# codelion/adaptive-classifier

Hardware: AMD Instinct MI355X
Metric: predict() queries/sec + kNN GB/s vs HBM roofline, 768-d (higher is better)
Workload: dtype f32

## Files before the change

### adaptive-classifier_amd/csrc/bert.hip

```cpp
#include "common.h"
#include "attention_core.h"

#include <math.h>
#include <atomic>
#include <chrono>
#include <string.h>

namespace {

typedef float f32x4 __attribute__((ext_vector_type(4)));
constexpr int kMaxVec = 8;

__device__ __forceinline__ float wave_sum(float v) {
#pragma unroll
    for (int o = 1; o < 64; o <<= 1) v += __shfl_xor(v, o);
    return v;
}

template <bool F16 = false>
__device__ __forceinline__ void layernorm_store(f32x4 (&x)[kMaxVec], int H, int lane, const float* g,
                                                const float* b, float eps, float* dst, uint16_t* planes = nullptr,
                                                int64_t rows = 0, int64_t row = 0) {
    const int nv = H >> 2;
    float s = 0.f;
// ... 4 lines not shown
    float q = 0.f;
#pragma unroll
    for (int e = 0; e < kMaxVec; ++e)
        if (lane + 64 * e < nv) {
            const float d0 = x[e].x - mean, d1 = x[e].y - mean, d2 = x[e].z - mean, d3 = x[e].w - mean;
            q += (d0 * d0 + d1 * d1) + (d2 * d2 + d3 * d3);
        }
    const float var = wave_sum(q) / (float)H;
    const float rstd = 1.0f / sqrtf(var + eps);
#pragma unroll
    for (int e = 0; e < kMaxVec; ++e) {
        const int c4 = lane + 64 * e;
        if (c4 < nv) {
            const f32x4 gg = *reinterpret_cast<const f32x4*>(g + 4 * c4);
            const f32x4 bb = *reinterpret_cast<const f32x4*>(b + 4 * c4);
            f32x4 y;
            y.x = (x[e].x - mean) * rstd * gg.x + bb.x;
            y.y = (x[e].y - mean) * rstd * gg.y + bb.y;
            y.z = (x[e].z - mean) * rstd * gg.z + bb.z;
            y.w = (x[e].w - mean) * rstd * gg.w + bb.w;
            *reinterpret_cast<f32x4*>(dst + 4 * c4) = y;
            if (planes)
                ac::emit_planes4(planes + ac::plane_off(rows, row, 4 * c4), rows * (int64_t)H, y, F16);
        }
    }
}

template <bool F16>
__global__ __launch_bounds__(256) void embed_ln_kernel(const int64_t* ids, const int64_t* type_ids, int T, int S,
                                                       int H, const float* word, const float* pos,
                                                       const float* type, const float* g, const float* b,
                                                       float eps, float* out, uint16_t* planes,
                                                       const int32_t* __restrict__ tok_src = nullptr,
                                                       const int32_t* __restrict__ t_dev = nullptr) {
    if (t_dev) T = t_dev[0];
    const int lane = threadIdx.x & 63;
    const int t = blockIdx.x * 4 + (threadIdx.x >> 6);
    if (t >= T) return;
    const int src = tok_src ? tok_src[t] : t;
    const int64_t id = ids[src];
    const int64_t tt = type_ids ? type_ids[src] : 0;
    const int p = src % S;
    const int nv = H >> 2;
    f32x4 x[kMaxVec];
#pragma unroll
    for (int e = 0; e < kMaxVec; ++e) {
        const int c4 = lane + 64 * e;
        if (c4 < nv) {
            const f32x4 w = *reinterpret_cast<const f32x4*>(word + id * H + 4 * c4);
            if (type) {
                const f32x4 ty = *reinterpret_cast<const f32x4*>(type + tt * H + 4 * c4);
                const f32x4 po = *reinterpret_cast<const f32x4*>(pos + (int64_t)p * H + 4 * c4);
                x[e] = (w + ty) + po;
            } else {
                x[e] = w;
            }
        }
    }
    layernorm_store<F16>(x, H, lane, g, b, eps, out + (int64_t)t * H, planes, T, t);
}

template <bool F16>
__global__ __launch_bounds__(256) void ln_kernel_t(const float* in, int T, int H, const float* g, const float* b,
                                                   float eps, float* out, uint16_t* planes, int64_t in_stride) {
    const int lane = threadIdx.x & 63;
    const int t = blockIdx.x * 4 + (threadIdx.x >> 6);
    if (t >= T) return;
// ... 582 lines not shown
    return AC_OK;
}

}

extern "C" int ac_bert_workspace(const ac_bert_config* cfg, int b, int S, size_t* bytes) {
    int rc = check_cfg(cfg);
    if (rc) return rc;
    AC_REQUIRE(bytes && b >= 0 && S >= 1, AC_EINVAL, "bert workspace: bad arguments");
    *bytes = bert_ws(*cfg, b > 0 ? b : 1, S).total;
    return AC_OK;
}

namespace {

static bool tail_fused() {
    const char* e = getenv("AC_BERT_TAIL_FUSED");
    return !(e && atoi(e) == 0);
}
inline bool pools_mean(int pool_opt) { return pool_opt == AC_POOL_MEAN; }
inline int token_layers(const ac_bert_config& c) { return pools_mean(c.pool_opt) ? c.layers : c.layers - 1; }
struct EncodePlan { bool wplanes, pl, f16; };
EncodePlan encode_plan(const ac_bert_config& c, const ac_bert_weights* w, int T) {
    const int H = c.hidden, I = c.intermediate;
    EncodePlan p;
    p.wplanes = w->qkv_w3 && w->ao_w3 && w->ff1_w3 && w->ff2_w3;
    p.pl = p.wplanes && ac::linear_takes_planes(T, H, H) && ac::linear_takes_planes(T, H, I) && (H % 8) == 0;
    p.f16 = p.pl && ac::gemm_arith() == AC_GEMM_F16X2 && w->qkv_wh && w->ao_wh && w->ff1_wh && w->ff2_wh && token_layers(c) > 0 &&
            ac::linear_f16x2_takes(T, 3 * H, H) && ac::linear_f16x2_takes(T, H, H) && ac::linear_f16x2_takes(T, I, H) &&
            ac::linear_f16x2_takes(T, H, I);
    return p;
}
void launch_embed(const ac_bert_config& c, const ac_bert_weights* w, const EncodePlan& pn, const int64_t* d_ids, const int64_t* d_type_ids,
                  int rows, int S, float* x, uint16_t* xp, const int32_t* tok_src, const int32_t* t_dev, hipStream_t stream) {
    const int H = c.hidden, tok_blocks = (rows + 3) / 4;
    if (pn.f16)
        hipLaunchKernelGGL(embed_ln_kernel<true>, dim3(tok_blocks), dim3(256), 0, stream, d_ids, d_type_ids, rows, S, H,
                           w->word_emb, w->pos_emb, w->type_emb, w->emb_ln_g, w->emb_ln_b, c.ln_eps, x, xp, tok_src, t_dev);
    else
        hipLaunchKernelGGL(embed_ln_kernel<false>, dim3(tok_blocks), dim3(256), 0, stream, d_ids, d_type_ids, rows, S, H,
                           w->word_emb, w->pos_emb, w->type_emb, w->emb_ln_g, w->emb_ln_b, c.ln_eps, x,
                           pn.pl ? xp : nullptr, tok_src, t_dev);
}
constexpr int kPreCtl = 1, kPreEmbed = 2;
int bert_encode_impl(const ac_bert_config* cfg, const ac_bert_weights* w, const int64_t* d_ids, const int64_t* d_type_ids,
                     const int64_t* d_mask, int b, int S, const int32_t* cu, const int32_t* tok_src, int T, int Smax,
                     float* d_out, int64_t ldo, void* d_ws, size_t ws_bytes, hipStream_t stream, int pre = 0) {
    int rc;
    const ac_bert_config& c = *cfg;
    const BertWs ws = bert_ws(c, b, S);
    AC_REQUIRE(d_ws && ws_bytes >= ws.total, AC_EWORKSPACE, "bert_encode_cls: workspace %zu < %zu", ws_bytes, ws.total);
    char* base = (char*)d_ws;
    float* x = (float*)(base + ws.x);
    float* qkv = (float*)(base + ws.qkv);
    float* ctx = (float*)(base + ws.ctx);
    float* y = (float*)(base + ws.y);
    float* ffn = (float*)(base + ws.ffn);
    const int H = c.hidden, I = c.intermediate;

    uint16_t* xp = (uint16_t*)(base + ws.xp);
    uint16_t* ctxp = (uint16_t*)(base + ws.ctxp);
    uint16_t* ffnp = (uint16_t*)(base + ws.ffnp);
    const EncodePlan pn = encode_plan(c, w, T);
    const bool wplanes = pn.wplanes, pl = pn.pl;
    const bool f16 = pn.f16;
    const bool pool = pools_mean(c.pool_opt);
    const bool fuse_ln = pl && token_layers(c) > 0 && ac::pipe_ln_applies(T, H, H) && ac::pipe_ln_applies(T, H, I);
    unsigned* ln_abort = (unsigned*)base;
    if (!(pre & kPreCtl)) {
        hipLaunchKernelGGL(ln_verdict_roll_kernel, dim3(1), dim3(1), 0, stream, ln_abort);
        AC_LAUNCH_CHECK();
    }
    unsigned* ln_count = (unsigned*)(base + ws.lnctl);
    const int ln_panels = ac::pipe_ln_panels(T);
    if (fuse_ln && !(pre & kPreCtl)) AC_HIP_CHECK(hipMemsetAsync(base + ws.lnctl, 0, ws.lnctl_bytes, stream));

    if (!(pre & kPreEmbed)) {
        launch_embed(c, w, pn, d_ids, d_type_ids, T, S, x, xp, tok_src, nullptr, stream);
        AC_LAUNCH_CHECK();
    }
    const int dh = c.hidden / c.heads;
    const float scale = 1.0f / sqrtf((float)dh);
    const int32_t* cu_at = cu;
    const bool fuse_attn = pl && token_layers(c) > 0 && dh == 64 && (cu || !d_mask) && ac::qkv_attn_applies(T, H, c.heads, Smax);
    if (fuse_attn && !cu) {
        int32_t* cuw = (int32_t*)(base + ws.cu);
        hipLaunchKernelGGL(iota_cu_kernel, dim3((b + 256) / 256), dim3(256), 0, stream, cuw, b, S);
        AC_LAUNCH_CHECK();
        cu_at = cuw;
    }
    int32_t* tile_seq = (int32_t*)(base + ws.tile_seq);
    unsigned* attn_xchg = nullptr;
    if (fuse_attn) {
        if (!(pre & kPreCtl) || !cu) {
            rc = ac::qkv_attn_tile_seq(cu_at, b, T, tile_seq, stream);
            if (rc) return rc;
        }
        if (ac::qkv_attn_exchange_applies(T, c.heads, (int)f16)) {
            attn_xchg = (unsigned*)(base + ws.attn_xchg);
            if (!(pre & kPreCtl)) AC_HIP_CHECK(hipMemsetAsync(attn_xchg, 0, ws.attn_xchg_bytes, stream));
        }
    }
    for (int l = 0; l < c.layers; ++l) {
        const uint16_t* qkv_w3 = wplanes ? w->qkv_w3[l] : nullptr;
        const uint16_t* ao_w3 = wplanes ? w->ao_w3[l] : nullptr;
        const uint16_t* ff1_w3 = wplanes ? w->ff1_w3[l] : nullptr;
        const uint16_t* ff2_w3 = wplanes ? w->ff2_w3[l] : nullptr;
        const bool last = (l == c.layers - 1) && !pool;
        const int Ml = last ? b : T;
        const bool lp = pl && !last;
        const float* resid = x;
// ... 25 lines not shown
            rc = ac::linear_f32_splitk(resid, ldres, w->qkv_w[l], H, w->qkv_b[l], nullptr, 0, y, H, b, H, H, 0, qkv_w3, ctx,
                                       (size_t)T * H * sizeof(float), stream, 3 * H);
        } else {
            rc = f16 ? ac::linear_f16x2(xp, w->qkv_wh[l], w->qkv_b[l], nullptr, 0, qkv, 3 * H, nullptr, T, 3 * H, H, 0, stream)
                     : ac::linear_f32(x, H, w->qkv_w[l], H, w->qkv_b[l], nullptr, 0, qkv, 3 * H, T, 3 * H, H, 0, nullptr, 1.f,
                                      stream, 0.f, 0, qkv_w3, pl ? xp : nullptr);
        }
        if (rc) return rc;
        if (fuse_attn && !last) {
        } else if (last) {
            const float* qc = q_cls_only ? y : nullptr;
            if (dh == 64 && Smax <= 32)
                hipLaunchKernelGGL((attention_cls_kernel<false, 64, 32>), dim3(c.heads, b), dim3(64), 0, stream, qkv, d_mask, S, H, scale,
                                   ctx, nullptr, nullptr, -1, cu, qc);
            else if (dh == 64)
                hipLaunchKernelGGL((attention_cls_kernel<false, 64>), dim3(c.heads, b), dim3(64), 0, stream, qkv, d_mask, S, H, scale,
                                   ctx, nullptr, nullptr, -1, cu, qc);
            else
                hipLaunchKernelGGL((attention_cls_kernel<false, 32>), dim3(c.heads, b), dim3(64), 0, stream, qkv, d_mask, S, H, scale,
                                   ctx, nullptr, nullptr, -1, cu, qc);
        } else {
            if (dh == 64)
                hipLaunchKernelGGL((attention_mfma_kernel<false, 64>), dim3((Smax + 31) / 32, c.heads, b), dim3(64), 0, stream, qkv,
                                   d_mask, S, H, scale, ctx, lp ? ctxp : nullptr, nullptr, nullptr, -1, cu, (int64_t)T, (int)f16);
            else
                hipLaunchKernelGGL((attention_mfma_kernel<false, 32>), dim3((Smax + 31) / 32, c.heads, b), dim3(64), 0, stream, qkv,
                                   d_mask, S, H, scale, ctx, lp ? ctxp : nullptr, nullptr, nullptr, -1, cu, (int64_t)T, (int)f16);
        }
        AC_LAUNCH_CHECK();
        const int lblocks = (Ml + 3) / 4;
        const bool fl = fuse_ln && lp;
        if (fl) {
            rc = ac::launch_gemm_pipe_ln(ctxp, Ml, f16 ? w->ao_wh[l] : ao_w3, H, w->ao_b[l], x, H, x, H, Ml, H, H, w->ln1_g[l], w->ln1_b[l], c.ln_eps,
                                         base + ws.lnpart, ln_count + (size_t)(2 * l) * ln_panels, ln_abort, xp, stream, (int)f16);
            if (rc) return rc;
        } else {
            rc = last ? ac::linear_f32_splitk(ctx, H, w->ao_w[l], H, w->ao_b[l], resid, ldres, y, H, Ml, H, H, 0, ao_w3, qkv,
                                              (size_t)T * 3 * H * sizeof(float), stream)
                      : (f16 ? ac::linear_f16x2(ctxp, w->ao_wh[l], w->ao_b[l], resid, ldres, y, H, nullptr, Ml, H, H, 0, stream)
                             : ac::linear_f32(ctx, H, w->ao_w[l], H, w->ao_b[l], resid, ldres, y, H, Ml, H, H, 0, nullptr, 1.f, stream,
                                              0.f, 0, ao_w3, lp ? ctxp : nullptr));
            if (rc) return rc;
            launch_ln(f16, lblocks, stream, y, Ml, H, w->ln1_g[l], w->ln1_b[l], c.ln_eps, last ? ctx : x, lp ? xp : nullptr, (int64_t)H);
            AC_LAUNCH_CHECK();
        }
        float* x1 = last ? ctx : x;
        rc = last ? ac::linear_f32_splitk(x1, H, w->ff1_w[l], H, w->ff1_b[l], nullptr, 0, ffn, I, Ml, I, H, 2, ff1_w3, qkv,
                                          (size_t)T * 3 * H * sizeof(float), stream)
                  : (f16 ? ac::linear_f16x2(xp, w->ff1_wh[l], w->ff1_b[l], nullptr, 0, nullptr, I, ffnp, Ml, I, H, 2, stream)
                         : ac::linear_f32(x1, H, w->ff1_w[l], H, w->ff1_b[l], nullptr, 0, ffn, I, Ml, I, H, 2, nullptr, 1.f, stream,
                                          0.f, 0, ff1_w3, lp ? xp : nullptr, lp ? ffnp : nullptr));
        if (rc) return rc;
        if (fl) {
            rc = ac::launch_gemm_pipe_ln(ffnp, Ml, f16 ? w->ff2_wh[l] : ff2_w3, H, w->ff2_b[l], x, H, x, H, Ml, H, I, w->ln2_g[l], w->ln2_b[l], c.ln_eps,
                                         base + ws.lnpart, ln_count + (size_t)(2 * l + 1) * ln_panels, ln_abort, xp, stream, (int)f16);
            if (rc) return rc;
            continue;
        }
        if (last && tail_fused()) {
            int ks = 0;
            rc = ac::linear_f32_splitk(ffn, I, w->ff2_w[l], I, w->ff2_b[l], x1, H, y, H, Ml, H, I, 0, ff2_w3, qkv,
                                       (size_t)T * 3 * H * sizeof(float), stream, 0, &ks);
            if (rc) return rc;
            if (ks > 0) {
                hipLaunchKernelGGL(splitk_ln_normalize_kernel, dim3(b), dim3(64), 0, stream, qkv, ks, b, H, w->ff2_b[l], x1, (int64_t)H,
                                   w->ln2_g[l], w->ln2_b[l], c.ln_eps, d_out, ldo);
                AC_LAUNCH_CHECK();
                return AC_OK;
            }
            launch_ln(f16, lblocks, stream, y, Ml, H, w->ln2_g[l], w->ln2_b[l], c.ln_eps, x, nullptr, (int64_t)H);
            AC_LAUNCH_CHECK();
            break;
        }
        rc = last ? ac::linear_f32_splitk(ffn, I, w->ff2_w[l], I, w->ff2_b[l], x1, H, y, H, Ml, H, I, 0, ff2_w3, qkv,
                                          (size_t)T * 3 * H * sizeof(float), stream)
                  : (f16 ? ac::linear_f16x2(ffnp, w->ff2_wh[l], w->ff2_b[l], x1, H, y, H, nullptr, Ml, H, I, 0, stream)
                         : ac::linear_f32(ffn, I, w->ff2_w[l], I, w->ff2_b[l], x1, H, y, H, Ml, H, I, 0, nullptr, 1.f, stream, 0.f, 0,
                                          ff2_w3, lp ? ffnp : nullptr));
        if (rc) return rc;
        launch_ln(f16, lblocks, stream, y, Ml, H, w->ln2_g[l], w->ln2_b[l], c.ln_eps, x, lp ? xp : nullptr, (int64_t)H);
        AC_LAUNCH_CHECK();
    }
    if (pool) {
        hipLaunchKernelGGL(pool_mean_normalize_kernel<false>, dim3(b), dim3(256), 3 * (size_t)H * sizeof(float), stream, x, d_mask, cu, S, H,
                           (const float*)nullptr, (const float*)nullptr, 0.f, d_out, ldo);
        AC_LAUNCH_CHECK();
        return AC_OK;
    }
// ... 89 lines not shown
    *epoch_out = (int)(n & 0x3fffffff) + 1;
    return base ? base + 16 * (n & 63) : nullptr;
}
}

static std::atomic<long long> g_unpad_wait_ns{0};
extern "C" long long ac_bert_unpad_last_wait_ns(void) { return g_unpad_wait_ns.load(std::memory_order_relaxed); }

extern "C" int ac_bert_encode_cls_unpad(const ac_bert_config* cfg, const ac_bert_weights* w, const int64_t* d_ids,
                                        const int64_t* d_type_ids, const int64_t* d_mask, int b, int S, float* d_out, int64_t ldo,
                                        void* d_ws, size_t ws_bytes, int clear_verdict, int* total_tokens, int* path, ac_stream_t stream_) {
    if (total_tokens) *total_tokens = 0;
    if (path) *path = AC_BERT_PATH_PACKED;
    int rc = check_cfg(cfg);
    if (rc) return rc;
    if (b == 0) return AC_OK;
    hipStream_t stream = (hipStream_t)stream_;
    const ac::CallScope scope(cfg->gemm_arith_opt, cfg->ln_fusion_opt, cfg->one_launch_opt);
    AC_REQUIRE(w && d_ids && d_mask && d_out && b > 0 && S >= 2 && S <= cfg->max_pos && ldo >= cfg->hidden && (int64_t)b * S > 32 &&
                   (int64_t)b * S < ((int64_t)1 << 30),
               AC_EINVAL, "bert_encode_cls_unpad: bad arguments (b=%d S=%d max_pos=%d; more than 32 token rows)", b, S, cfg->max_pos);
    const ac_bert_config& c = *cfg;
    const BertWs ws = bert_ws(c, b, S);
    AC_REQUIRE(d_ws && ws_bytes >= ws.total, AC_EWORKSPACE, "bert_encode_cls_unpad: workspace %zu < %zu", ws_bytes, ws.total);
    char* base = (char*)d_ws;
    int32_t* cu = (int32_t*)(base + ws.cu);
    int32_t* src = (int32_t*)(base + ws.pack_src);
    int32_t* info = (int32_t*)(base + ws.pack_info);
    int epoch = 0;
    int32_t* slot = info_slot(&epoch);
    const size_t lds = (size_t)(2 * b + 1) * sizeof(int32_t);
    AC_REQUIRE(slot && lds <= 96 * 1024, AC_EUNSUPPORTED, "bert_encode_cls_unpad: %d sequences in one call (or no pinned host memory): "
               "use ac_bert_pack + ac_bert_encode_cls_packed", b);
    if (lds > 48 * 1024) (void)hipFuncSetAttribute((const void*)pack_prologue_kernel, hipFuncAttributeMaxDynamicSharedMemorySize, (int)lds);
    hipLaunchKernelGGL(pack_prologue_kernel, dim3(1), dim3(1024), lds, stream, d_mask, b, S, cu, src, info, (int32_t*)(base + ws.tile_seq),
                       (unsigned*)(base + ws.lnctl), (int)(ws.lnctl_bytes / 4), (unsigned*)(base + ws.attn_xchg), (int)(ws.attn_xchg_bytes / 4),
                       (unsigned*)base, clear_verdict, slot, epoch);
    AC_LAUNCH_CHECK();
    const EncodePlan lo = encode_plan(c, w, b), hi = encode_plan(c, w, b * S);
    const bool early = lo.pl == hi.pl && lo.f16 == hi.f16;
    if (early) {
        launch_embed(c, w, hi, d_ids, d_type_ids, b * S, S, (float*)(base + ws.x), (uint16_t*)(base + ws.xp), src, info, stream);
        AC_LAUNCH_CHECK();
    }
    volatile int32_t* vs = slot;
    bool seen = false;
    const auto wait_t0 = std::chrono::steady_clock::now();
    for (int spin = 0; spin < 200000 && !seen; ++spin) {
        seen = __atomic_load_n(&vs[3], __ATOMIC_ACQUIRE) == epoch;
        if (!seen) __builtin_ia32_pause();
    }
    if (!seen) {
        AC_HIP_CHECK(hipStreamSynchronize(stream));
        seen = __atomic_load_n(&vs[3], __ATOMIC_ACQUIRE) == epoch;
        AC_REQUIRE(seen, AC_EHIP, "bert_encode_cls_unpad: the packing kernel's report never arrived");
    }
    g_unpad_wait_ns.store(std::chrono::duration_cast<std::chrono::nanoseconds>(std::chrono::steady_clock::now() - wait_t0).count(),
                          std::memory_order_relaxed);
    const int total = vs[0], not_prefix = vs[1], longest = vs[2];
    if (total_tokens) *total_tokens = total;
    if (!not_prefix && total < b * S) {
        AC_REQUIRE(total >= b && longest >= 1 && longest <= S, AC_EHIP, "bert_encode_cls_unpad: bad report (%d rows, longest %d)", total, longest);
        return bert_encode_impl(cfg, w, d_ids, d_type_ids, nullptr, b, S, cu, src, total, longest, d_out, ldo, d_ws, ws_bytes, stream,
                                kPreCtl | (early ? kPreEmbed : 0));
    }
    if (path) *path = not_prefix ? AC_BERT_PATH_PADDED_MASK : AC_BERT_PATH_PADDED;
    if (total_tokens) *total_tokens = b * S;
    return bert_encode_impl(cfg, w, d_ids, d_type_ids, not_prefix ? d_mask : nullptr, b, S, nullptr, nullptr, b * S, S, d_out, ldo, d_ws,
                            ws_bytes, stream);
}

extern "C" int ac_bert_encode_cls_packed(const ac_bert_config* cfg, const ac_bert_weights* w, const int64_t* d_ids,
                                         const int64_t* d_type_ids, int b, int S, const int32_t* d_cu,
                                         const int32_t* d_tok_src, int total_tokens, int longest, float* d_out, int64_t ldo,
                                         void* d_ws, size_t ws_bytes, ac_stream_t stream_) {
// ... 194 lines not shown
```

### adaptive-classifier_amd/csrc/common.h

```cpp
#pragma once
#include <atomic>
#include <hip/hip_runtime.h>
#include <stdarg.h>
#include <stdint.h>
#include <stdio.h>

#include "../../include/acamd.h"

namespace ac {

void set_error(const char* fmt, ...);

struct DevInfo {
    int cus;
    int lds_per_block;
    size_t hbm_bytes;
    int hw_cus;
};
const DevInfo& dev_info();

bool test_hooks_enabled();
#define AC_TEST_HOOK_ONLY(name)                                                                                                   \
    do {                                                                                                                          \
        if (!ac::test_hooks_enabled()) {                                                                                          \
// ... 16 lines not shown

#define AC_REQUIRE(cond, code, ...)                                                     \
    do {                                                                                \
        if (!(cond)) {                                                                  \
            ac::set_error(__VA_ARGS__);                                                 \
            return (code);                                                              \
        }                                                                               \
    } while (0)

#define AC_LAUNCH_CHECK()                                                               \
    do {                                                                                \
        hipError_t _e = hipGetLastError();                                              \
        if (_e != hipSuccess) {                                                         \
            ac::set_error("kernel launch failed: %s (%s:%d)", hipGetErrorString(_e),    \
                          __FILE__, __LINE__);                                          \
            return AC_EHIP;                                                             \
        }                                                                               \
    } while (0)

__host__ __device__ static inline size_t align_up(size_t x, size_t a) { return (x + a - 1) / a * a; }
static inline int next_pow2(int x) { int p = 1; while (p < x) p <<= 1; return p; }

int linear_f32(const float* A, int64_t lda, const float* W, int64_t ldw, const float* bias,
               const float* residual, int64_t ldr, float* C, int64_t ldc, int M, int N, int K, int act,
               const uint8_t* mask, float mask_scale, hipStream_t stream, float drop_p = 0.f,
               uint64_t drop_seed = 0, const uint16_t* W_planes = nullptr, const uint16_t* A_planes = nullptr,
               uint16_t* C_planes = nullptr, int64_t w_plane_rows = 0);
int linear_f32_splitk(const float* A, int64_t lda, const float* W, int64_t ldw, const float* bias, const float* residual,
                      int64_t ldr, float* C, int64_t ldc, int M, int N, int K, int act, const uint16_t* W_planes, float* scratch,
                      size_t scratch_bytes, hipStream_t stream, int64_t w_plane_rows = 0, int* partials_only = nullptr);
bool pipe_ln_applies(int M, int N, int K);
size_t pipe_ln_part_bytes(int M, int N);
int pipe_ln_panels(int M);
int launch_gemm_pipe_ln(const uint16_t* Ap, int64_t a_rows, const uint16_t* Wp, int64_t w_rows, const float* bias,
                        const float* residual, int64_t ldr, float* C, int64_t ldc, int M, int N, int K, const float* gamma,
                        const float* beta, float eps, void* part, unsigned* count, unsigned* abort_flag, uint16_t* planes,
                        hipStream_t stream, int f16 = 0);
constexpr int kQkvAttnRows = 256;
constexpr int kQkvAttnCu = 264;
bool qkv_attn_applies(int M, int H, int heads, int smax);
size_t qkv_attn_tile_seq_bytes(int M);
int qkv_attn_tile_seq(const int32_t* cu, int b, int M, int32_t* tile_seq, hipStream_t stream);
bool qkv_attn_exchange_applies(int M, int heads, int f16);
int launch_gemm_pipe_qkv_attn(const uint16_t* Ap, int64_t a_rows, const uint16_t* Wp, int64_t w_rows, const float* bias, int M, int H,
                              int heads, const int32_t* cu, const int32_t* tile_seq, int b, int smax, float scale, uint16_t* ctx_planes,
                              float* qkv, hipStream_t stream, int f16 = 0, unsigned* exchange = nullptr, unsigned epoch = 0,
                              unsigned* abort_flag = nullptr);
bool linear_takes_planes(int M, int N, int K);

__host__ __device__ static inline bool dropout_keep(uint64_t seed, uint64_t idx, float p) {
    uint64_t z = seed + idx * 0x9E3779B97F4A7C15ull;
    z = (z ^ (z >> 30)) * 0xBF58476D1CE4E5B9ull;
    z = (z ^ (z >> 27)) * 0x94D049BB133111EBull;
    z ^= z >> 31;
    return (float)(z >> 40) * (1.0f / 16777216.0f) >= p;
}
#ifdef __HIPCC__
typedef __bf16 bf16x2_t __attribute__((ext_vector_type(2)));
typedef float f32x2_t __attribute__((ext_vector_type(2)));
typedef float f32x4_t __attribute__((ext_vector_type(4)));

__device__ __forceinline__ uint32_t pack_bf16(float a, float b) {
    const f32x2_t f = {a, b};
    return __builtin_bit_cast(uint32_t, __builtin_convertvector(f, bf16x2_t));
}
__device__ __forceinline__ void split2(float a, float b, uint32_t& h, uint32_t& m, uint32_t& l) {
    h = pack_bf16(a, b);
    const float ra = a - __uint_as_float(h << 16), rb = b - __uint_as_float(h & 0xffff0000u);
    m = pack_bf16(ra, rb);
    const float sa = ra - __uint_as_float(m << 16), sb = rb - __uint_as_float(m & 0xffff0000u);
// ... 244 lines not shown
```

### adaptive-classifier_amd/csrc/gemm_common.h

```cpp
#pragma once
#include "common.h"
#include "gemm_plan.h"

#include <math.h>

namespace acg {

typedef float f32x4 __attribute__((ext_vector_type(4)));
typedef float f32x16 __attribute__((ext_vector_type(16)));

struct Epilogue {
    const float* bias = nullptr;
    const float* residual = nullptr;
    int64_t ldr = 0;
    int act = ACT_NONE;
    float alpha = 1.f;
    float beta = 0.f;
    const uint8_t* mask = nullptr;
    float mask_scale = 1.f;
    uint64_t drop_seed = 0;
    float drop_p = 0.f;
    const float* gate = nullptr;
    int64_t ldg = 0;
    float gate_scale = 1.f;
};

struct LnFuse {
    const float* gamma;
    const float* beta;
    float eps;
    float2* part;
    unsigned* count;
    unsigned* abort_;
    uint16_t* planes;
    int starve;
    int fences;
};

struct AttnFuse {
    const int32_t* cu;
    const int32_t* tile_seq;
    int b, H, smax;
    float scale;
    uint16_t* ctx_planes;
    float* qkv;
    unsigned* exchange;
    unsigned epoch;
    int fences;
    unsigned* abort_;
};

__device__ __forceinline__ float apply_epilogue(const Epilogue& e, float acc, int64_t row, int col,
                                                const float* C, int64_t ldc, int N) {
    float v = e.alpha * acc;
    if (e.beta != 0.f) v = fmaf(e.beta, C[row * ldc + col], v);
    if (e.bias) v += e.bias[col];
    if (e.act == ACT_RELU) v = v < 0.f ? 0.f : v;
    else if (e.act == ACT_GELU) v = ac::gelu_erf(v);
    if (e.mask) v = e.mask[row * (int64_t)N + col] ? v * e.mask_scale : 0.f;
    else if (e.drop_p > 0.f) v = ac::dropout_keep(e.drop_seed, (uint64_t)(row * (int64_t)N + col), e.drop_p) ? v * e.mask_scale : 0.f;
    if (e.residual) v += e.residual[row * e.ldr + col];
    if (e.gate) v = (e.gate[row * e.ldg + col] != 0.f) ? v * e.gate_scale : 0.f;
    return v;
}

template <int EPI>
__device__ __forceinline__ float fast_epilogue(float acc, float bias, float res) {
    if (EPI == EPI_IDENT) return acc;
// ... 132 lines not shown
```

### adaptive-classifier_amd/csrc/gemm_pipe.hip

```cpp
#include "common.h"
#include "gemm_common.h"
#include "grid_sync.h"
#include "attention_core.h"

#include <stdio.h>
#include <stdlib.h>

#include <atomic>
#include <type_traits>

namespace {
using namespace acg;

constexpr int PSBK = 16;

struct PipeParams {
    const uint16_t* Ap; int64_t a_rows;
    const uint16_t* Wp; int64_t w_rows;
    float* C; int64_t ldc;
    int M, N, K;
    Epilogue epi;
    LnFuse ln;
    AttnFuse at;
    unsigned long long* stamps;
    int krot;
};

template <int STRIDE = 4>
__device__ __forceinline__ void stamp(const PipeParams& prm, int wave, int i) {
    if (prm.stamps && wave == 0) {
        const unsigned long long t = clock64();
        if ((threadIdx.x & 63) == 0) prm.stamps[(size_t)blockIdx.x * STRIDE + i] = t;
    }
}

template <int N> __device__ __forceinline__ void wait_vm() {
    static_assert(N >= 0 && N <= 63, "vmcnt immediate");
    asm volatile("s_waitcnt vmcnt(%0)" ::"n"(N) : "memory");
}
// ... 37 lines not shown
    static_assert(BM <= 64 * NW, "one thread per tile row in the combine steps");
    const Epilogue& e = prm.epi;
    const LnFuse& ln = prm.ln;
    float2* wstat = reinterpret_cast<float2*>(lds_f + NW * kTrFloats);
    float2* rstat = wstat + WNW * BM;
    unsigned* okf = reinterpret_cast<unsigned*>(rstat + BM);
    const int m0 = bm * BM, n0 = bn * BN, c = lane & 31;
#pragma unroll
    for (int mi = 0; mi < TM; ++mi)
#pragma unroll
        for (int ni = 0; ni < TN; ++ni) {
            const float bias = e.bias[n0 + wn * WC + ni * 32 + c];
#pragma unroll
            for (int r = 0; r < 16; ++r) acc[mi][ni][r] = (acc[mi][ni][r] + bias) + res[(mi * TN + ni) * 16 + r];
        }
#pragma unroll
    for (int mi = 0; mi < TM; ++mi)
#pragma unroll
        for (int r = 0; r < 16; ++r) {
            float s = 0.f;
#pragma unroll
            for (int ni = 0; ni < TN; ++ni) s += acc[mi][ni][r];
            s = acp::row16_sum(s);
            s += __shfl_xor(s, 16);
            const float mw = s * (1.0f / WC);
            float q = 0.f;
#pragma unroll
            for (int ni = 0; ni < TN; ++ni) { const float d = acc[mi][ni][r] - mw; q = fmaf(d, d, q); }
            q = acp::row16_sum(q);
            q += __shfl_xor(q, 16);
            if (c == r) wstat[wn * BM + wm * (32 * TM) + mi * 32 + acc_row32(r, lane)] = make_float2(mw, q);
        }
    __syncthreads();
    if (tid < BM) {
        float mean = 0.f;
#pragma unroll
        for (int w = 0; w < WNW; ++w) mean += wstat[w * BM + tid].x;
        mean *= 1.0f / WNW;
        float m2 = 0.f;
#pragma unroll
        for (int w = 0; w < WNW; ++w) { const float2 pw = wstat[w * BM + tid]; const float d = pw.x - mean; m2 += fmaf((float)WC * d, d, pw.y); }
        const unsigned long long bits = (unsigned long long)__float_as_uint(mean) | ((unsigned long long)__float_as_uint(m2) << 32);
        __hip_atomic_store(reinterpret_cast<unsigned long long*>(ln.part + ((size_t)bm * ntn + bn) * BM + tid), bits,
                           __ATOMIC_RELAXED, __HIP_MEMORY_SCOPE_AGENT);
    }
    asm volatile("s_waitcnt vmcnt(0)" ::: "memory");
    __syncthreads();
    if (tid == 0) {
        if (ln.fences) __hip_atomic_fetch_add(ln.count + bm, 1u, __ATOMIC_RELEASE, __HIP_MEMORY_SCOPE_AGENT);
        else __hip_atomic_fetch_add(ln.count + bm, 1u, __ATOMIC_RELAXED, __HIP_MEMORY_SCOPE_AGENT);
    }
    if (tid < 64) {
        unsigned ok = 1;
        for (long spins = 0;; ++spins) {
            const unsigned v = __hip_atomic_load(ln.count + bm, __ATOMIC_RELAXED, __HIP_MEMORY_SCOPE_AGENT);
            if (v >= (unsigned)(ntn + ln.starve)) {
                if (ln.fences) __builtin_amdgcn_fence(__ATOMIC_ACQUIRE, "agent");
                else asm volatile("" ::: "memory");
                break;
            }
            __builtin_amdgcn_s_sleep(1);
            if ((spins & 63) == 63 && (spins > (1l << 20) || __hip_atomic_load(ln.abort_, __ATOMIC_RELAXED, __HIP_MEMORY_SCOPE_AGENT))) {
                if (lane == 0) __hip_atomic_store(ln.abort_, 1u, __ATOMIC_RELAXED, __HIP_MEMORY_SCOPE_AGENT);
                ok = 0;
                break;
            }
        }
        if (lane == 0) *okf = ok;
    }
    __syncthreads();
    if (tid < BM) {
        float2 pj[8];
        const float* base = reinterpret_cast<const float*>(ln.part + (size_t)bm * ntn * BM + tid);
#pragma unroll
        for (int j = 0; j < 8; ++j) pj[j] = j < ntn ? acp::ld2_sc1(base + (size_t)j * BM * 2) : make_float2(0.f, 0.f);
        float mean = 0.f;
#pragma unroll
        for (int j = 0; j < 8; ++j) mean += pj[j].x;
        mean /= (float)ntn;
        float m2 = 0.f;
#pragma unroll
        for (int j = 0; j < 8; ++j) if (j < ntn) { const float d = pj[j].x - mean; m2 += fmaf((float)BN * d, d, pj[j].y); }
        const float var = m2 / (float)prm.N;
        const float rstd = 1.0f / sqrtf(var + ln.eps);
        rstat[tid] = make_float2(mean, *okf ? rstd : __uint_as_float(0x7fc00000u));
    }
    __syncthreads();
#pragma unroll
    for (int mi = 0; mi < TM; ++mi)
#pragma unroll
        for (int ni = 0; ni < TN; ++ni) {
            const int col = n0 + wn * WC + ni * 32 + c;
            const float g = ln.gamma[col], b = ln.beta[col];
#pragma unroll
            for (int r = 0; r < 16; ++r) {
                const float2 st = rstat[wm * (32 * TM) + mi * 32 + acc_row32(r, lane)];
                acc[mi][ni][r] = (acc[mi][ni][r] - st.x) * st.y * g + b;
            }
        }
    store_tile<EPI_IDENT, TM, BM, TN>(acc, prm.C, prm.ldc, prm.M, prm.N, m0, n0, wm, wn, lane, e);
    if (ln.planes)
        store_tile_planes<EPI_IDENT, TM, TN, AR>(acc, ln.planes, prm.M, prm.N, m0, n0, wm, wn, lane, e, lds_f + wave * kTrFloats);
}

constexpr int kAtLd = 196;
constexpr int kAtRows = 160;
constexpr int kAtCu = ac::kQkvAttnCu;
constexpr int kAtBytes = kAtRows * kAtLd * 4 + kAtCu * 4;

template <int TM, int TN, int WMW, int WNW, int AR>
__device__ __forceinline__ void qkv_attention_epilogue(f32x16 (&acc)[TM][TN], const PipeParams& prm, int bm, int head, int wm, int wn,
                                                       int lane, int wave, float* T, int cu_pref, const float (&bias)[TN]) {
    static_assert(TM == 2 && TN == 3 && WMW == 4 && WNW == 2, "built for the 256 x 192 tile (8 waves of 64 x 96)");
    constexpr int BM = 256, NW = WMW * WNW;
    const AttnFuse& at = prm.at;
    const int m0 = bm * BM, H = at.H, c = lane & 31;
    const int stride = at.smax <= 32 ? 128 : 96;
    const int tile_end = m0 + BM < prm.M ? m0 + BM : prm.M;
// ... 492 lines not shown
    p.Ap = Ap; p.a_rows = a_rows; p.Wp = Wp; p.w_rows = w_rows; p.C = qkv; p.ldc = 3 * (int64_t)H; p.M = M; p.N = 3 * H; p.K = H;
    p.epi.bias = bias;
    p.at.cu = cu; p.at.tile_seq = tile_seq; p.at.b = b; p.at.H = H; p.at.smax = smax; p.at.scale = scale; p.at.ctx_planes = ctx_planes;
    p.at.qkv = qkv;
    AC_REQUIRE(!exchange || (abort_flag && qkv_attn_exchange_applies(M, heads, f16)), AC_EINVAL,
               "gemm_pipe_qkv_attn: the in-launch exchange needs every tile resident (%d rows x %d heads) and an abort word", M, heads);
    p.at.exchange = exchange; p.at.epoch = epoch; p.at.abort_ = abort_flag; p.at.fences = exchange_fences();
    g_qkv_attn_launches.fetch_add(1, std::memory_order_relaxed);
    return f16 ? launch_one<EPI_QKV_ATTN, 2, 3, 4, 2, 4, false, 2, 2>(p, stream)
               : launch_one<EPI_QKV_ATTN, 2, 3, 4, 2, 3, false, 2, 3>(p, stream);
}

static std::atomic<int> g_ln_fusion{-1};
static std::atomic<long long> g_ln_launches{0};
bool ln_fusion_enabled() {
    if (const int o = call_opts().ln_fusion; o >= 0) return o != 0;
    int v = g_ln_fusion.load(std::memory_order_relaxed);
    if (v < 0) {
        const char* e = getenv("AC_LN_FUSION");
        v = (e && atoi(e) == 0) ? 0 : 1;
        g_ln_fusion.store(v, std::memory_order_relaxed);
    }
    return v != 0;
}
static int64_t ln_resident_capacity() {
    using G = PipeGeom<1, 2, 4, 2, 6, 3>;
    constexpr int LN_BYTES = G::TR_BYTES + (2 + 1) * G::BM * 8 + 16;
    return resident_capacity(OCC_LN, (const void*)gemm_pipe_nt<EPI_BIAS_RES_LN, 1, 2, 4, 2, 6, false, 2, 3>, 64 * G::NW,
                             G::LDS_BYTES > LN_BYTES ? G::LDS_BYTES : LN_BYTES);
}
bool pipe_ln_applies(int M, int N, int K) {
    return ln_fusion_enabled() && pipe_ln_shape(M, N, K, gemm_env()) && tiles_of(M, N, kLnBM, kLnBN) <= ln_resident_capacity();
}
size_t pipe_ln_part_bytes(int M, int N) { return (size_t)((M + kLnBM - 1) / kLnBM) * (size_t)(N / kLnBN) * kLnBM * sizeof(float2); }
int pipe_ln_panels(int M) { return (M + kLnBM - 1) / kLnBM; }

int launch_gemm_pipe_ln(const uint16_t* Ap, int64_t a_rows, const uint16_t* Wp, int64_t w_rows, const float* bias,
                        const float* residual, int64_t ldr, float* C, int64_t ldc, int M, int N, int K, const float* gamma,
                        const float* beta, float eps, void* part, unsigned* count, unsigned* abort_flag, uint16_t* planes,
                        hipStream_t stream, int f16) {
    AC_REQUIRE(pipe_ln_applies(M, N, K), AC_EUNSUPPORTED, "gemm_pipe: fused LayerNorm epilogue not applicable to %d x %d x %d", M, N, K);
    AC_REQUIRE(Ap && Wp && bias && residual && C && gamma && beta && part && count && abort_flag, AC_EINVAL, "gemm_pipe_ln: null pointer");
    PipeParams p{};
    p.Ap = Ap; p.a_rows = a_rows; p.Wp = Wp; p.w_rows = w_rows; p.C = C; p.ldc = ldc; p.M = M; p.N = N; p.K = K;
    p.epi.bias = bias; p.epi.residual = residual; p.epi.ldr = ldr;
    p.ln.gamma = gamma; p.ln.beta = beta; p.ln.eps = eps; p.ln.part = (float2*)part; p.ln.count = count; p.ln.abort_ = abort_flag;
    p.ln.fences = exchange_fences();
    p.ln.planes = planes; p.ln.starve = (call_opts().ln_fusion >= 0 ? call_opts().ln_fusion : g_ln_fusion.load(std::memory_order_relaxed)) == 2 ? 1 : 0;
    g_ln_launches.fetch_add(1, std::memory_order_relaxed);
    return f16 ? launch_cfg<1, 2, 4, 2, 6, 2, 2>(EPI_BIAS_RES_LN, false, p, stream)
               : launch_cfg<1, 2, 4, 2, 6, 2>(EPI_BIAS_RES_LN, false, p, stream);
}
}

extern "C" int ac_gemm_set_ln_fusion(int on) {
    AC_TEST_HOOK_ONLY("ac_gemm_set_ln_fusion");
    ac::g_ln_fusion.store(on == 2 ? 2 : (on ? 1 : 0), std::memory_order_relaxed);
    return AC_OK;
}

extern "C" int64_t ac_gemm_ln_fusion_launches(void) { return (int64_t)ac::g_ln_launches.load(std::memory_order_relaxed); }
extern "C" int64_t ac_gemm_qkv_attn_launches(void) { return (int64_t)ac::g_qkv_attn_launches.load(std::memory_order_relaxed); }

static int parse_pipe_table(const char* spec, acg::PipeTable* t) {
    if (!spec) { t->n = -1; return AC_OK; }
    int n = 0;
    const char* p = spec;
    while (*p && n < 16) {
        int N = 0, K = 0, cfg = 0, used = 0;
        if (sscanf(p, "%dx%d=%d%n", &N, &K, &cfg, &used) != 3) { ac::set_error("gemm pipe table: cannot parse '%s'", p); return AC_EINVAL; }
        t->rules[n++] = {N, K, cfg};
        p += used;
        if (*p == ';') ++p;
    }
    t->n = n;
    return AC_OK;
}
extern "C" int ac_gemm_set_pipe_table(const char* spec) {
    AC_TEST_HOOK_ONLY("ac_gemm_set_pipe_table");
    return parse_pipe_table(spec, &ac::g_pipe_table);
// ... 6 lines not shown
```

Before: 54980.

## Replace LN cross-tile counter barrier with tagged self-validating stat granules

The fused LayerNorm GEMM epilogue used to publish per-tile row statistics, bump a per-panel atomic counter, then spin until every tile had arrived before reading all partials. By default it now writes each statistic as a 64-bit granule with a per-launch tag in the high bits and polls only the peers' granules until their tags match. This removes the counter atomic, the vmcnt wait and two block barriers. Because the tags are distinct per launch, the per-call memset of the counter buffer is no longer needed; the partial buffer is cleared inside the embedding kernel instead. In exchange the partial buffer doubles in size, and correctness depends on 64-bit relaxed atomic stores being visible without fences, which is why the old path is kept when fences are on or an environment flag selects it.

After: 55080 (median of 6 runs). No clear change (+0.2%).

```diff
diff --git a/adaptive-classifier_amd/csrc/bert.hip b/adaptive-classifier_amd/csrc/bert.hip
--- a/adaptive-classifier_amd/csrc/bert.hip
+++ b/adaptive-classifier_amd/csrc/bert.hip
@@ -60,7 +60,13 @@
                                                        const float* type, const float* g, const float* b,
                                                        float eps, float* out, uint16_t* planes,
                                                        const int32_t* __restrict__ tok_src = nullptr,
-                                                       const int32_t* __restrict__ t_dev = nullptr) {
+                                                       const int32_t* __restrict__ t_dev = nullptr,
+                                                       uint4* __restrict__ zero16 = nullptr, int64_t zero_n = 0) {
+    if (zero16) {
+        const int64_t per = (zero_n + (int64_t)gridDim.x - 1) / (int64_t)gridDim.x;
+        const int64_t hi = ((int64_t)blockIdx.x + 1) * per, end = hi < zero_n ? hi : zero_n;
+        for (int64_t i = (int64_t)blockIdx.x * per + threadIdx.x; i < end; i += 256) zero16[i] = make_uint4(0u, 0u, 0u, 0u);
+    }
     if (t_dev) T = t_dev[0];
     const int lane = threadIdx.x & 63;
     const int t = blockIdx.x * 4 + (threadIdx.x >> 6);
@@ -709,15 +715,17 @@
     return p;
 }
 void launch_embed(const ac_bert_config& c, const ac_bert_weights* w, const EncodePlan& pn, const int64_t* d_ids, const int64_t* d_type_ids,
-                  int rows, int S, float* x, uint16_t* xp, const int32_t* tok_src, const int32_t* t_dev, hipStream_t stream) {
+                  int rows, int S, float* x, uint16_t* xp, const int32_t* tok_src, const int32_t* t_dev, void* ln_part, hipStream_t stream) {
     const int H = c.hidden, tok_blocks = (rows + 3) / 4;
+    uint4* z = (uint4*)ln_part;
+    const int64_t zn = ln_part ? (int64_t)(ac::pipe_ln_part_bytes(rows, H) / sizeof(uint4)) : 0;
     if (pn.f16)
         hipLaunchKernelGGL(embed_ln_kernel<true>, dim3(tok_blocks), dim3(256), 0, stream, d_ids, d_type_ids, rows, S, H,
-                           w->word_emb, w->pos_emb, w->type_emb, w->emb_ln_g, w->emb_ln_b, c.ln_eps, x, xp, tok_src, t_dev);
+                           w->word_emb, w->pos_emb, w->type_emb, w->emb_ln_g, w->emb_ln_b, c.ln_eps, x, xp, tok_src, t_dev, z, zn);
     else
         hipLaunchKernelGGL(embed_ln_kernel<false>, dim3(tok_blocks), dim3(256), 0, stream, d_ids, d_type_ids, rows, S, H,
                            w->word_emb, w->pos_emb, w->type_emb, w->emb_ln_g, w->emb_ln_b, c.ln_eps, x,
-                           pn.pl ? xp : nullptr, tok_src, t_dev);
+                           pn.pl ? xp : nullptr, tok_src, t_dev, z, zn);
 }
 constexpr int kPreCtl = 1, kPreEmbed = 2;
 int bert_encode_impl(const ac_bert_config* cfg, const ac_bert_weights* w, const int64_t* d_ids, const int64_t* d_type_ids,
@@ -750,10 +758,11 @@
     }
     unsigned* ln_count = (unsigned*)(base + ws.lnctl);
     const int ln_panels = ac::pipe_ln_panels(T);
-    if (fuse_ln && !(pre & kPreCtl)) AC_HIP_CHECK(hipMemsetAsync(base + ws.lnctl, 0, ws.lnctl_bytes, stream));
+    const bool ln_flag = ac::ln_exchange_flag();
+    if (fuse_ln && ln_flag && !(pre & kPreCtl)) AC_HIP_CHECK(hipMemsetAsync(base + ws.lnctl, 0, ws.lnctl_bytes, stream));
 
     if (!(pre & kPreEmbed)) {
-        launch_embed(c, w, pn, d_ids, d_type_ids, T, S, x, xp, tok_src, nullptr, stream);
+        launch_embed(c, w, pn, d_ids, d_type_ids, T, S, x, xp, tok_src, nullptr, fuse_ln && !ln_flag ? base + ws.lnpart : nullptr, stream);
         AC_LAUNCH_CHECK();
     }
     const int dh = c.hidden / c.heads;
@@ -845,7 +854,8 @@
         const bool fl = fuse_ln && lp;
         if (fl) {
             rc = ac::launch_gemm_pipe_ln(ctxp, Ml, f16 ? w->ao_wh[l] : ao_w3, H, w->ao_b[l], x, H, x, H, Ml, H, H, w->ln1_g[l], w->ln1_b[l], c.ln_eps,
-                                         base + ws.lnpart, ln_count + (size_t)(2 * l) * ln_panels, ln_abort, xp, stream, (int)f16);
+                                         base + ws.lnpart, ln_count + (size_t)(2 * l) * ln_panels, ln_abort, xp, stream, (int)f16,
+                                         ln_flag ? 0u : (unsigned)(2 * l + 1));
             if (rc) return rc;
         } else {
             rc = last ? ac::linear_f32_splitk(ctx, H, w->ao_w[l], H, w->ao_b[l], resid, ldres, y, H, Ml, H, H, 0, ao_w3, qkv,
@@ -866,7 +876,8 @@
         if (rc) return rc;
         if (fl) {
             rc = ac::launch_gemm_pipe_ln(ffnp, Ml, f16 ? w->ff2_wh[l] : ff2_w3, H, w->ff2_b[l], x, H, x, H, Ml, H, I, w->ln2_g[l], w->ln2_b[l], c.ln_eps,
-                                         base + ws.lnpart, ln_count + (size_t)(2 * l + 1) * ln_panels, ln_abort, xp, stream, (int)f16);
+                                         base + ws.lnpart, ln_count + (size_t)(2 * l + 1) * ln_panels, ln_abort, xp, stream, (int)f16,
+                                         ln_flag ? 0u : (unsigned)(2 * l + 2));
             if (rc) return rc;
             continue;
         }
@@ -1022,15 +1033,17 @@
     const size_t lds = (size_t)(2 * b + 1) * sizeof(int32_t);
     AC_REQUIRE(slot && lds <= 96 * 1024, AC_EUNSUPPORTED, "bert_encode_cls_unpad: %d sequences in one call (or no pinned host memory): "
                "use ac_bert_pack + ac_bert_encode_cls_packed", b);
+    const bool ln_flag = ac::ln_exchange_flag();
     if (lds > 48 * 1024) (void)hipFuncSetAttribute((const void*)pack_prologue_kernel, hipFuncAttributeMaxDynamicSharedMemorySize, (int)lds);
     hipLaunchKernelGGL(pack_prologue_kernel, dim3(1), dim3(1024), lds, stream, d_mask, b, S, cu, src, info, (int32_t*)(base + ws.tile_seq),
-                       (unsigned*)(base + ws.lnctl), (int)(ws.lnctl_bytes / 4), (unsigned*)(base + ws.attn_xchg), (int)(ws.attn_xchg_bytes / 4),
+                       (unsigned*)(base + ws.lnctl), ln_flag ? (int)(ws.lnctl_bytes / 4) : 0, (unsigned*)(base + ws.attn_xchg), (int)(ws.attn_xchg_bytes / 4),
                        (unsigned*)base, clear_verdict, slot, epoch);
     AC_LAUNCH_CHECK();
     const EncodePlan lo = encode_plan(c, w, b), hi = encode_plan(c, w, b * S);
     const bool early = lo.pl == hi.pl && lo.f16 == hi.f16;
     if (early) {
-        launch_embed(c, w, hi, d_ids, d_type_ids, b * S, S, (float*)(base + ws.x), (uint16_t*)(base + ws.xp), src, info, stream);
+        launch_embed(c, w, hi, d_ids, d_type_ids, b * S, S, (float*)(base + ws.x), (uint16_t*)(base + ws.xp), src, info,
+                     ln_flag ? nullptr : base + ws.lnpart, stream);
         AC_LAUNCH_CHECK();
     }
     volatile int32_t* vs = slot;
diff --git a/adaptive-classifier_amd/csrc/common.h b/adaptive-classifier_amd/csrc/common.h
--- a/adaptive-classifier_amd/csrc/common.h
+++ b/adaptive-classifier_amd/csrc/common.h
@@ -72,10 +72,11 @@
 bool pipe_ln_applies(int M, int N, int K);
 size_t pipe_ln_part_bytes(int M, int N);
 int pipe_ln_panels(int M);
+bool ln_exchange_flag();
 int launch_gemm_pipe_ln(const uint16_t* Ap, int64_t a_rows, const uint16_t* Wp, int64_t w_rows, const float* bias,
                         const float* residual, int64_t ldr, float* C, int64_t ldc, int M, int N, int K, const float* gamma,
                         const float* beta, float eps, void* part, unsigned* count, unsigned* abort_flag, uint16_t* planes,
-                        hipStream_t stream, int f16 = 0);
+                        hipStream_t stream, int f16, unsigned tag);
 constexpr int kQkvAttnRows = 256;
 constexpr int kQkvAttnCu = 264;
 bool qkv_attn_applies(int M, int H, int heads, int smax);
diff --git a/adaptive-classifier_amd/csrc/gemm_common.h b/adaptive-classifier_amd/csrc/gemm_common.h
--- a/adaptive-classifier_amd/csrc/gemm_common.h
+++ b/adaptive-classifier_amd/csrc/gemm_common.h
@@ -34,6 +34,7 @@
     unsigned* abort_;
     uint16_t* planes;
     int starve;
+    unsigned tag;
     int fences;
 };
 
diff --git a/adaptive-classifier_amd/csrc/gemm_pipe.hip b/adaptive-classifier_amd/csrc/gemm_pipe.hip
--- a/adaptive-classifier_amd/csrc/gemm_pipe.hip
+++ b/adaptive-classifier_amd/csrc/gemm_pipe.hip
@@ -5,6 +5,7 @@
 
 #include <stdio.h>
 #include <stdlib.h>
+#include <string.h>
 
 #include <atomic>
 #include <type_traits>
@@ -108,48 +109,15 @@
             if (c == r) wstat[wn * BM + wm * (32 * TM) + mi * 32 + acc_row32(r, lane)] = make_float2(mw, q);
         }
     __syncthreads();
+    float t_mean = 0.f, t_m2 = 0.f;
     if (tid < BM) {
-        float mean = 0.f;
-#pragma unroll
-        for (int w = 0; w < WNW; ++w) mean += wstat[w * BM + tid].x;
-        mean *= 1.0f / WNW;
-        float m2 = 0.f;
-#pragma unroll
-        for (int w = 0; w < WNW; ++w) { const float2 pw = wstat[w * BM + tid]; const float d = pw.x - mean; m2 += fmaf((float)WC * d, d, pw.y); }
-        const unsigned long long bits = (unsigned long long)__float_as_uint(mean) | ((unsigned long long)__float_as_uint(m2) << 32);
-        __hip_atomic_store(reinterpret_cast<unsigned long long*>(ln.part + ((size_t)bm * ntn + bn) * BM + tid), bits,
-                           __ATOMIC_RELAXED, __HIP_MEMORY_SCOPE_AGENT);
-    }
-    asm volatile("s_waitcnt vmcnt(0)" ::: "memory");
-    __syncthreads();
-    if (tid == 0) {
-        if (ln.fences) __hip_atomic_fetch_add(ln.count + bm, 1u, __ATOMIC_RELEASE, __HIP_MEMORY_SCOPE_AGENT);
-        else __hip_atomic_fetch_add(ln.count + bm, 1u, __ATOMIC_RELAXED, __HIP_MEMORY_SCOPE_AGENT);
-    }
-    if (tid < 64) {
-        unsigned ok = 1;
-        for (long spins = 0;; ++spins) {
-            const unsigned v = __hip_atomic_load(ln.count + bm, __ATOMIC_RELAXED, __HIP_MEMORY_SCOPE_AGENT);
-            if (v >= (unsigned)(ntn + ln.starve)) {
-                if (ln.fences) __builtin_amdgcn_fence(__ATOMIC_ACQUIRE, "agent");
-                else asm volatile("" ::: "memory");
-                break;
-            }
-            __builtin_amdgcn_s_sleep(1);
-            if ((spins & 63) == 63 && (spins > (1l << 20) || __hip_atomic_load(ln.abort_, __ATOMIC_RELAXED, __HIP_MEMORY_SCOPE_AGENT))) {
-                if (lane == 0) __hip_atomic_store(ln.abort_, 1u, __ATOMIC_RELAXED, __HIP_MEMORY_SCOPE_AGENT);
-                ok = 0;
-                break;
-            }
-        }
-        if (lane == 0) *okf = ok;
-    }
-    __syncthreads();
-    if (tid < BM) {
-        float2 pj[8];
-        const float* base = reinterpret_cast<const float*>(ln.part + (size_t)bm * ntn * BM + tid);
-#pragma unroll
-        for (int j = 0; j < 8; ++j) pj[j] = j < ntn ? acp::ld2_sc1(base + (size_t)j * BM * 2) : make_float2(0.f, 0.f);
+#pragma unroll
+        for (int w = 0; w < WNW; ++w) t_mean += wstat[w * BM + tid].x;
+        t_mean *= 1.0f / WNW;
+#pragma unroll
+        for (int w = 0; w < WNW; ++w) { const float2 pw = wstat[w * BM + tid]; const float d = pw.x - t_mean; t_m2 += fmaf((float)WC * d, d, pw.y); }
+    }
+    auto combine = [&](const float2 (&pj)[8], bool ok) {
         float mean = 0.f;
 #pragma unroll
         for (int j = 0; j < 8; ++j) mean += pj[j].x;
@@ -159,7 +127,92 @@
         for (int j = 0; j < 8; ++j) if (j < ntn) { const float d = pj[j].x - mean; m2 += fmaf((float)BN * d, d, pj[j].y); }
         const float var = m2 / (float)prm.N;
         const float rstd = 1.0f / sqrtf(var + ln.eps);
-        rstat[tid] = make_float2(mean, *okf ? rstd : __uint_as_float(0x7fc00000u));
+        rstat[tid] = make_float2(mean, ok ? rstd : __uint_as_float(0x7fc00000u));
+    };
+    if (ln.tag != 0u) {
+        if (tid < BM) {
+            unsigned long long* gran = reinterpret_cast<unsigned long long*>(ln.part);
+            const unsigned long long tag_hi = (unsigned long long)ln.tag << 32;
+            unsigned long long* mine = gran + (((size_t)bm * ntn + bn) * BM + tid) * 2;
+            __hip_atomic_store(mine, tag_hi | __float_as_uint(t_mean), __ATOMIC_RELAXED, __HIP_MEMORY_SCOPE_AGENT);
+            __hip_atomic_store(mine + 1, tag_hi | __float_as_uint(t_m2), __ATOMIC_RELAXED, __HIP_MEMORY_SCOPE_AGENT);
+            const unsigned want = ln.starve ? (ln.tag | 0x80000000u) : ln.tag;
+            const unsigned long long* row = gran + ((size_t)bm * ntn * BM + tid) * 2;
+            float2 pj[8];
+            unsigned stale = 0u;
+#pragma unroll
+            for (int j = 0; j < 8; ++j) {
+                pj[j] = make_float2(0.f, 0.f);
+                if (j < ntn) {
+                    if (j == bn && !ln.starve) pj[j] = make_float2(t_mean, t_m2);
+                    else stale |= 1u << j;
+                }
+            }
+            bool ok = true;
+            for (long spins = 0; stale != 0u; ++spins) {
+                unsigned long long g0[8], g1[8];
+#pragma unroll
+                for (int j = 0; j < 8; ++j) {
+                    g0[j] = 0ull; g1[j] = 0ull;
+                    if (stale & (1u << j)) {
+                        g0[j] = __hip_atomic_load(row + (size_t)j * BM * 2, __ATOMIC_RELAXED, __HIP_MEMORY_SCOPE_AGENT);
+                        g1[j] = __hip_atomic_load(row + (size_t)j * BM * 2 + 1, __ATOMIC_RELAXED, __HIP_MEMORY_SCOPE_AGENT);
+                    }
+                }
+#pragma unroll
+                for (int j = 0; j < 8; ++j)
+                    if ((stale & (1u << j)) && (unsigned)(g0[j] >> 32) == want && (unsigned)(g1[j] >> 32) == want) {
+                        pj[j] = make_float2(__uint_as_float((unsigned)g0[j]), __uint_as_float((unsigned)g1[j]));
+                        stale &= ~(1u << j);
+                    }
+                if (stale == 0u) break;
+                __builtin_amdgcn_s_sleep(1);
+                if ((spins & 63) == 63 && (spins > (1l << 20) || __hip_atomic_load(ln.abort_, __ATOMIC_RELAXED, __HIP_MEMORY_SCOPE_AGENT))) {
+                    __hip_atomic_store(ln.abort_, 1u, __ATOMIC_RELAXED, __HIP_MEMORY_SCOPE_AGENT);
+                    ok = false;
+                    break;
+                }
+            }
+            combine(pj, ok);
+        }
+    } else {
+        if (tid < BM) {
+            const unsigned long long bits = (unsigned long long)__float_as_uint(t_mean) | ((unsigned long long)__float_as_uint(t_m2) << 32);
+            __hip_atomic_store(reinterpret_cast<unsigned long long*>(ln.part + ((size_t)bm * ntn + bn) * BM + tid), bits,
+                               __ATOMIC_RELAXED, __HIP_MEMORY_SCOPE_AGENT);
+        }
+        asm volatile("s_waitcnt vmcnt(0)" ::: "memory");
+        __syncthreads();
+        if (tid == 0) {
+            if (ln.fences) __hip_atomic_fetch_add(ln.count + bm, 1u, __ATOMIC_RELEASE, __HIP_MEMORY_SCOPE_AGENT);
+            else __hip_atomic_fetch_add(ln.count + bm, 1u, __ATOMIC_RELAXED, __HIP_MEMORY_SCOPE_AGENT);
+        }
+        if (tid < 64) {
+            unsigned ok = 1;
+            for (long spins = 0;; ++spins) {
+                const unsigned v = __hip_atomic_load(ln.count + bm, __ATOMIC_RELAXED, __HIP_MEMORY_SCOPE_AGENT);
+                if (v >= (unsigned)(ntn + ln.starve)) {
+                    if (ln.fences) __builtin_amdgcn_fence(__ATOMIC_ACQUIRE, "agent");
+                    else asm volatile("" ::: "memory");
+                    break;
+                }
+                __builtin_amdgcn_s_sleep(1);
+                if ((spins & 63) == 63 && (spins > (1l << 20) || __hip_atomic_load(ln.abort_, __ATOMIC_RELAXED, __HIP_MEMORY_SCOPE_AGENT))) {
+                    if (lane == 0) __hip_atomic_store(ln.abort_, 1u, __ATOMIC_RELAXED, __HIP_MEMORY_SCOPE_AGENT);
+                    ok = 0;
+                    break;
+                }
+            }
+            if (lane == 0) *okf = ok;
+        }
+        __syncthreads();
+        if (tid < BM) {
+            float2 pj[8];
+            const float* base = reinterpret_cast<const float*>(ln.part + (size_t)bm * ntn * BM + tid);
+#pragma unroll
+            for (int j = 0; j < 8; ++j) pj[j] = j < ntn ? acp::ld2_sc1(base + (size_t)j * BM * 2) : make_float2(0.f, 0.f);
+            combine(pj, *okf != 0u);
+        }
     }
     __syncthreads();
 #pragma unroll
@@ -718,20 +771,26 @@
 bool pipe_ln_applies(int M, int N, int K) {
     return ln_fusion_enabled() && pipe_ln_shape(M, N, K, gemm_env()) && tiles_of(M, N, kLnBM, kLnBN) <= ln_resident_capacity();
 }
-size_t pipe_ln_part_bytes(int M, int N) { return (size_t)((M + kLnBM - 1) / kLnBM) * (size_t)(N / kLnBN) * kLnBM * sizeof(float2); }
+size_t pipe_ln_part_bytes(int M, int N) { return (size_t)((M + kLnBM - 1) / kLnBM) * (size_t)(N / kLnBN) * kLnBM * 2 * sizeof(unsigned long long); }
 int pipe_ln_panels(int M) { return (M + kLnBM - 1) / kLnBM; }
+bool ln_exchange_flag() {
+    if (exchange_fences()) return true;
+    const char* e = getenv("AC_LN_EXCHANGE");
+    return e && strcmp(e, "flag") == 0;
+}
 
 int launch_gemm_pipe_ln(const uint16_t* Ap, int64_t a_rows, const uint16_t* Wp, int64_t w_rows, const float* bias,
                         const float* residual, int64_t ldr, float* C, int64_t ldc, int M, int N, int K, const float* gamma,
                         const float* beta, float eps, void* part, unsigned* count, unsigned* abort_flag, uint16_t* planes,
-                        hipStream_t stream, int f16) {
+                        hipStream_t stream, int f16, unsigned tag) {
     AC_REQUIRE(pipe_ln_applies(M, N, K), AC_EUNSUPPORTED, "gemm_pipe: fused LayerNorm epilogue not applicable to %d x %d x %d", M, N, K);
     AC_REQUIRE(Ap && Wp && bias && residual && C && gamma && beta && part && count && abort_flag, AC_EINVAL, "gemm_pipe_ln: null pointer");
-    PipeParams p{};
+    AC_REQUIRE(tag < 0x80000000u, AC_EINVAL, "gemm_pipe_ln: granule tag %u out of range", tag);    PipeParams p{};
     p.Ap = Ap; p.a_rows = a_rows; p.Wp = Wp; p.w_rows = w_rows; p.C = C; p.ldc = ldc; p.M = M; p.N = N; p.K = K;
     p.epi.bias = bias; p.epi.residual = residual; p.epi.ldr = ldr;
     p.ln.gamma = gamma; p.ln.beta = beta; p.ln.eps = eps; p.ln.part = (float2*)part; p.ln.count = count; p.ln.abort_ = abort_flag;
     p.ln.fences = exchange_fences();
+    p.ln.tag = tag;
     p.ln.planes = planes; p.ln.starve = (call_opts().ln_fusion >= 0 ? call_opts().ln_fusion : g_ln_fusion.load(std::memory_order_relaxed)) == 2 ? 1 : 0;
     g_ln_launches.fetch_add(1, std::memory_order_relaxed);
     return f16 ? launch_cfg<1, 2, 4, 2, 6, 2, 2>(EPI_BIAS_RES_LN, false, p, stream)
```
